# Plonky3/Plonky3-recursion

Measured on AMD Instinct MI355X. Metric: prove_next_layer ms + Poseidon2 perms/s, KoalaBear 2^20-row circuit, 1/8 GPU, lower is better.
Workload: dtype u32 Montgomery (31-bit prime field, degree-4 extension); Poseidon2 hashing as exact integers in f64; 1 GPU; prove_next_layer (verifier-circuit run on the device + prove_all_tables) of the synthetic koala-bear 2^20-row recursion layer: tables const/public/alu/poseidon2/recompose, FRI blowup 4, arity<=4, 54 queries, 15-bit PoW; circuit inputs + NextLayerPrepCache resident in HBM; field=koala-bear, log_height=20, independent_proofs=1, proof_bytes=612900, parallelism=1 independent proofs, one per GPU, no data-path collective

## Files before the change

__graft_entry__.py:

```python
import os
import subprocess
import sys
import time

ROOT = os.path.dirname(os.path.abspath(__file__))
CSRC = os.path.join(ROOT, "plonky3_recursion_amd", "csrc")
LIB = os.path.join(ROOT, "plonky3_recursion_amd", "libp3r_hip.so")
KNOBS_LIB = os.path.join(ROOT, "plonky3_recursion_amd", "knobs", "libp3r_hip.so")
HIP_SOURCES = ["p3r_core.hip", "tu_lde.hip", "tu_open.hip", "tu_fri.hip", "tu_air.hip", "tu_quotient.hip", "tu_logup.hip", "tu_mmcs4.hip", "prep_device.hip"]


def _stale(target, deps):
    if not os.path.exists(target):
        return True
    t = os.path.getmtime(target)
    return any(os.path.getmtime(d) > t for d in deps)


def _deps_of(obj):
    dep = obj + ".d"
    if not os.path.exists(dep):
        return None
    txt = open(dep).read().replace("\\\n", " ")
    return [p for p in txt.split(":", 1)[1].split() if p]


def build():
    hipcc = os.environ.get("HIPCC", "/opt/rocm/bin/hipcc")
    flags = ["-O3", "-std=c++17", "--offload-arch=gfx950", "-fPIC", "-pthread"]
    objdir = os.path.join(CSRC, ".build")
    os.makedirs(objdir, exist_ok=True)
    os.makedirs(os.path.dirname(KNOBS_LIB), exist_ok=True)
    shared = ["prep_device.hip", "tu_open.hip", "tu_fri.hip", "tu_air.hip", "tu_quotient.hip", "tu_logup.hip", "tu_mmcs4.hip"]
    knobbed = ["p3r_core.hip", "tu_lde.hip"]
    units = [(src, src + ".o", []) for src in HIP_SOURCES]
    units += [(src, src.replace(".hip", ".knobs.o"), ["-DP3R_TUNING_KNOBS"]) for src in knobbed]
    test_only = ["tu_prims_test.hip", "tu_p2f_test.hip", "tu_field_test.hip"]
    units += [(src, src.replace(".hip", ".knobs.o"), ["-DP3R_TUNING_KNOBS"]) for src in test_only]
    pending = []
    for src, objname, extra in units:
        obj = os.path.join(objdir, objname)
        deps = _deps_of(obj)
        if deps is None or not all(os.path.exists(d) for d in deps) or _stale(obj, deps):
            pending.append((obj, [hipcc] + flags + extra + ["-MD", "-MF", obj + ".d", "-c", "-o", obj, os.path.join(CSRC, src)]))
    pending.sort(key=lambda job: 0 if "p3r_core" in os.path.basename(job[0]) else 1)
    running, failed = [], None
    max_jobs = max(1, min(len(pending), (os.cpu_count() or 2)))
    while pending or running:
        while pending and len(running) < max_jobs:
            obj, cmd = pending.pop(0)
            running.append((obj, subprocess.Popen(cmd, cwd=CSRC)))
        done = [job for job in running if job[1].poll() is not None]
        if not done:
            time.sleep(0.2)
            continue
        obj, proc = done[0]
        running.remove(done[0])
        if proc.returncode != 0:
            for p in (obj, obj + ".d"):
                if os.path.exists(p):
                    os.remove(p)
            failed = failed or subprocess.CalledProcessError(proc.returncode, proc.args)
    if failed:
        raise failed
    for lib, objs in ((LIB, [s + ".o" for s in HIP_SOURCES]),
                      (KNOBS_LIB, [s.replace(".hip", ".knobs.o") for s in knobbed + test_only] + [s + ".o" for s in shared])):
        paths = [os.path.join(objdir, o) for o in objs]
        if _stale(lib, paths):
            subprocess.run([hipcc] + flags + ["-shared", "-o", lib] + paths, check=True, cwd=CSRC)
    subprocess.run(["make", "-C", os.path.join(ROOT, "oracle")], check=True,
                   stdout=subprocess.DEVNULL)
    subprocess.run(["make", "-C", os.path.join(ROOT, "harness")], check=True,
                   stdout=subprocess.DEVNULL, stderr=subprocess.DEVNULL)
    subprocess.run(["make", "-C", os.path.join(ROOT, "examples")], check=True, stdout=subprocess.DEVNULL)
    chk = os.path.join(ROOT, "tools", "microbench", "zk_fill_check")
    srcs = [chk + ".hip", os.path.join(CSRC, "kernels_zk.hip.h"), os.path.join(CSRC, "zk_rand.h")]
    if not os.path.exists(chk) or any(os.path.getmtime(f) > os.path.getmtime(chk) for f in srcs):
        subprocess.run([hipcc, "--offload-arch=gfx950", "-O3", "-std=c++17", "-w", "-I", CSRC, "-o", chk, chk + ".hip"], check=True)
    if ROOT not in sys.path:
        sys.path.insert(0, ROOT)
    import plonky3_recursion_amd
    from plonky3_recursion_amd import _lib
    _lib.load()


def smoke():
    if ROOT not in sys.path:
        sys.path.insert(0, ROOT)
    sys.path.insert(0, os.path.join(ROOT, "tests"))
    import numpy as np
# ... 66 lines not shown
```

plonky3_recursion_amd/csrc/kernels_fri_reduce.hip.h:

```cpp
#pragma once
#include "kernels_stark.hip.h"

namespace p3r {

template <int DC>
struct FriInvJobT {
  uint32_t* inv;
  uint64_t h;
  int log_h;
  uint32_t w_h;
  uint32_t w_4;
  EW<DC> z;
  uint32_t block0;
};
using FriInvJob = FriInvJobT<4>;
template <class PP, int DC = 4>
__global__ void __launch_bounds__(kBlock)
k_fri_inv_points(const FriInvJobT<DC>* __restrict__ jobs, int n_jobs, uint32_t gen) {
  using F = Fp<PP>;
  using E = typename Chal<PP, DC>::type;
  const int j = find_job(jobs, n_jobs);
  const FriInvJobT<DC>& job = jobs[j];
  const size_t h = job.h, r0 = ((size_t)(blockIdx.x - job.block0) * kBlock + threadIdx.x) * 4;
  if (r0 >= h) return;
  const E z = e4_load<PP, DC>(job.z);
  E x[4], v[4];
  const F x0 = F::raw(gen) * F::raw(job.w_h).pow(bit_reverse((uint32_t)r0, job.log_h));
  const F x2 = x0 * F::raw(job.w_4);
  x[0] = z - E::from_base(x0);
  x[1] = z + E::from_base(x0);
  x[2] = z - E::from_base(x2);
  x[3] = z + E::from_base(x2);
  inv4<PP>(x, v);
  const gptr<uint32_t> inv = as_global(job.inv);
#pragma unroll
  for (int m = 0; m < 4; ++m)
    if (r0 + m < h)
#pragma unroll
      for (int k = 0; k < DC; ++k) inv[(size_t)k * h + r0 + m] = v[m].c[k].v;
}

struct FriVsumJob {
  const uint32_t* vals;
  uint32_t* out;
  int w;
};
template <class PP, int DC = 4>
__global__ void __launch_bounds__(kBlock)
k_fri_vsum(const FriVsumJob* __restrict__ jobs, const uint32_t* __restrict__ apow_tab ) {
  using F = Fp<PP>;
  using E = typename Chal<PP, DC>::type;
  __shared__ uint32_t sh[kBlock / 64][DC];
  const FriVsumJob job = jobs[blockIdx.x];
  const gptr<const uint32_t> vals = as_global(job.vals);
  E acc = E::zero();
  for (int c = threadIdx.x; c < job.w; c += kBlock) {
    E ap, v;
#pragma unroll
    for (int k = 0; k < DC; ++k) {
      ap.c[k] = F::raw(apow_tab[DC * c + k]);
      v.c[k] = F::raw(vals[DC * c + k]);
    }
    acc += ap * v;
  }
  const int lane = threadIdx.x & 63, wave = threadIdx.x >> 6;
#pragma unroll
  for (int k = 0; k < DC; ++k) {
    F x = acc.c[k];
#pragma unroll
    for (int off = 32; off > 0; off >>= 1) x += F::raw(__shfl_down(x.v, off));
    if (lane == 0) sh[wave][k] = x.v;
  }
  __syncthreads();
  if (threadIdx.x < DC) {
    F x = F::zero();
#pragma unroll
    for (int wv = 0; wv < kBlock / 64; ++wv) x += F::raw(sh[wv][threadIdx.x]);
    as_global(job.out)[threadIdx.x] = x.v;
  }
}

template <int DC>
struct FriReduceMatT {
  const uint32_t* mat;
  int w, n_points;
  const uint32_t* inv[2];
  const uint32_t* v[2];
  EW<DC> off[2];
};
using FriReduceMat = FriReduceMatT<4>;
struct FriReduceJob {
  uint32_t* ro;
  uint64_t h;
  uint32_t mat0, n_mats;
  uint32_t block0;
};
template <class PP, int DC = 4>
__global__ void __launch_bounds__(kBlock)
k_fri_reduce_pre(const FriReduceJob* __restrict__ jobs, int n_jobs, const FriReduceMatT<DC>* __restrict__ mats,
                 const uint32_t* __restrict__ apow_tab ) {
  using F = Fp<PP>;
  using E = typename Chal<PP, DC>::type;
  const int j = find_job(jobs, n_jobs);
  const FriReduceJob job = jobs[j];
  const size_t h = job.h, r = (size_t)(blockIdx.x - job.block0) * kBlock + threadIdx.x;
  if (r >= h) return;
  auto apow = [&](int c) {
    E ap;
#pragma unroll
    for (int k = 0; k < DC; ++k) ap.c[k] = F::raw(apow_tab[DC * c + k]);
    return ap;
  };
  E acc = E::zero();
  for (uint32_t m = 0; m < job.n_mats; ++m) {
    const FriReduceMatT<DC>& a = mats[job.mat0 + m];
    const gptr<const uint32_t> mat = as_global(a.mat);
    const int w = a.w;
    E S = E::zero(), S2 = E::zero();
    int c = 0;
    for (; c + 3 < w; c += 4) {
      const F m0 = F::raw(mat[(size_t)c * h + r]), m1 = F::raw(mat[(size_t)(c + 1) * h + r]);
      const F m2 = F::raw(mat[(size_t)(c + 2) * h + r]), m3 = F::raw(mat[(size_t)(c + 3) * h + r]);
      S += E::dot2_base(apow(c), m0, apow(c + 1), m1);
      S2 += E::dot2_base(apow(c + 2), m2, apow(c + 3), m3);
    }
    for (; c + 1 < w; c += 2)
      S += E::dot2_base(apow(c), F::raw(mat[(size_t)c * h + r]), apow(c + 1), F::raw(mat[(size_t)(c + 1) * h + r]));
    if (c < w) S += apow(c) * F::raw(mat[(size_t)c * h + r]);
    S += S2;
    for (int p = 0; p < a.n_points; ++p) {
      E inv;
#pragma unroll
      for (int k = 0; k < DC; ++k) inv.c[k] = F::raw(as_global(a.inv[p])[(size_t)k * h + r]);
      E V;
#pragma unroll
      for (int k = 0; k < DC; ++k) V.c[k] = F::raw(as_global(a.v[p])[k]);
      acc += e4_load<PP, DC>(a.off[p]) * (V - S) * inv;
    }
  }
#pragma unroll
  for (int k = 0; k < DC; ++k) as_global(job.ro)[(size_t)k * h + r] = acc.c[k].v;
}

}
```

plonky3_recursion_amd/csrc/prove_impl.hip.h:

```cpp
#include "host_transcript.h"
#include "kernels_stark.hip.h"
#include "kernels_fri_reduce.hip.h"
#include "kernels_zk.hip.h"
#include "open_impl.hip.h"

struct p3r_prep {
  std::vector<p3r::AirParams> airs;
  std::vector<std::unique_ptr<p3r_dmat>> traces;
  std::vector<std::unique_ptr<p3r_dmat>> evals;
  std::vector<std::unique_ptr<p3r_dmat>> ldes;
  std::vector<size_t> heights;
  int zk_codewords = -1;
  const p3r_dmat* committed(size_t i) const { return evals.empty() ? traces[i].get() : evals[i].get(); }
  std::unique_ptr<p3r_tree> tree;
  std::vector<uint32_t> cap_canonical;
};

namespace {

template <class PP, int DC = 4>
EW<DC> to_e4(const typename Chal<PP, DC>::type& e) { return e4_store<PP, DC>(e); }

template <class PP, int DC = 4>
std::vector<typename Chal<PP, DC>::type> download_ef(p3r_ctx* ctx, const uint32_t* dev, size_t count) {
  std::vector<uint32_t> raw(count * DC);
  P3R_HIP(fetch_small(ctx, dev, raw.size(), raw.data()));
  std::vector<typename Chal<PP, DC>::type> out(count);
  for (size_t i = 0; i < count; ++i)
    for (int k = 0; k < DC; ++k) out[i].c[k] = Fp<PP>::raw(raw[i * DC + k]);
  return out;
}

inline ZkKey zk_key_of(const p3r_ctx* ctx, uint64_t nonce) {
  ZkKey k{};
  for (int i = 0; i < 8; ++i) k.k[i] = ctx->zk_key[i];
  k.nonce_lo = (uint32_t)nonce; k.nonce_hi = (uint32_t)(nonce >> 32);
  return k;
}

template <class PP>
void launch_zk_tiles(p3r_ctx* ctx, std::vector<ZkTileJob>& jobs, const ZkKey& key, const char* family) {
  uint64_t blocks = 0;
  for (auto& j : jobs) {
    if (2 * (uint64_t)(j.w2 | 1u) > kZkTileWords) fail(P3R_EUNSUPPORTED, "ZK fill of a matrix of %u columns", j.w2);
    j.log_tr = zk_tile_log_rows(j.rows, j.w2);
    j.block0 = (uint32_t)blocks;
    blocks += j.rows >> j.log_tr;
  }
  if (blocks >= (uint64_t(1) << 31)) fail(P3R_EUNSUPPORTED, "ZK fill launch of %llu tiles", (unsigned long long)blocks);
  if (!blocks) return;
  DevBuf d_jobs((jobs.size() * sizeof(ZkTileJob) + 3) / 4);
  P3R_HIP(ctx->stage.upload(ctx->stream, d_jobs.p, jobs.data(), jobs.size() * sizeof(ZkTileJob)));
  ProfScope ps(ctx, family);
  hipLaunchKernelGGL(k_zk_fill_tiles<PP>, dim3((unsigned)blocks), dim3(kBlock), 0, ctx->stream, reinterpret_cast<const ZkTileJob*>(d_jobs.p),
                     (int)jobs.size(), key);
// ... 196 lines not shown
  }
  std::vector<uint32_t> cap_mont;
  const ZkKey prep_key = zk_key_of(ctx, 0);
  prep->tree = lde_and_commit<PP>(ctx, items, (int)ctx->cfg.log_blowup, prep->ldes, cap_mont, kSaltRound + ZK_ROUND_PREP, &prep_key);
  prep->cap_canonical.resize(cap_mont.size());
  for (size_t i = 0; i < cap_mont.size(); ++i) prep->cap_canonical[i] = F::raw(cap_mont[i]).to_canonical();
  return prep;
}

template <class PP, int DC>
struct ProofRound {
  using E = typename Chal<PP, DC>::type;
  struct Mat {
    int inst;
    const p3r_dmat *ev, *lde;
    Fp<PP> shift;
    std::vector<E> z;
    size_t job = 0;
    std::vector<std::vector<E>> vals, codewords;
  };
  std::unique_ptr<p3r_tree> own;
  const p3r_tree* tree = nullptr;
  std::vector<uint32_t> cap;
  std::vector<std::unique_ptr<p3r_dmat>> keep, lde;
  std::vector<Mat> mats;
};

template <class PP, int DC>
struct BatchProver {
  using F = Fp<PP>;
  using E = typename Chal<PP, DC>::type;
  using Round = ProofRound<PP, DC>;
  using Mat = typename Round::Mat;
  static constexpr size_t kMaxPhases = 32;

  p3r_ctx* const ctx;
  const p3r_prep* const prep;
  const p3r_dmat* const* const mains;
  const size_t ni;
  const p3r_config& cfg;
  const int log_blowup;
  const int zk, R;
  const ZkKey zk_key;
  std::vector<LookupLayout> layouts;
  std::vector<int> log_n, log_e;
  const F gen = F::generator();
  std::vector<uint32_t> rc_mont;
  HostChallenger<PP, DC> ch;
  ProofWriter<PP, DC> W;
  Round main_round, perm_round, quot_round, rand_round, prep_round;
  LookupChT<DC> lc{};
  std::vector<E> terminals;
  E alpha, zeta;
  DevBuf d_apow, d_fapow;
  Opener<PP, DC> op;
  std::map<std::array<uint64_t, 6>, uint32_t*> inv_cache;
  std::vector<DevBuf> inv_keep;
  std::map<int, std::pair<E, DevBuf>> ros;
  struct Phase { int la; size_t rows; DevBuf folded_in; std::unique_ptr<p3r_tree> tree; std::vector<uint32_t> cap; };
  std::vector<Phase> phases;
  int log_max = 0;
  DevBuf folded, d_tstate, d_phase;
  std::vector<F> commit_pow_witnesses;
  std::vector<E> final_poly;
  F query_pow_witness;
  struct QPath { uint32_t at = 0; const p3r_tree* t = nullptr; };
  struct QRound { std::vector<std::pair<uint32_t, uint32_t>> rows; QPath path; uint32_t tree_shift; };
  struct QPhase { uint32_t sib_at[16]; QPath path; int shift; uint32_t salt_at = 0; };
  std::vector<size_t> indices;
  std::vector<QRound> qrounds;
  std::vector<QPhase> qphases;
  uint32_t words_per_query = 0;
  const uint32_t* gathered = nullptr;

  BatchProver(p3r_ctx* c, const p3r_prep* p, const p3r_dmat* const* m, size_t n, bool canonical_encoding)
      : ctx(c), prep(p), mains(m), ni(n), cfg(c->cfg), log_blowup((int)cfg.log_blowup), zk(cfg.zk ? 1 : 0), R(zk_codewords(cfg)),
        zk_key(zk_key_of(c, (zk || cfg.mmcs_salt_elems) ? c->zk_nonce++ : 0)),
        layouts(n), log_n(n), log_e(n), rc_mont(c->rc_canonical.size()), ch(rc_mont.data()), terminals(n, E::zero()),
        op(c) {
    const int p2w = p2_perm_cols<PP>() + 2;
    for (size_t i = 0; i < ni; ++i) {
      const AirParams& a = prep->airs[i];
      if (mains[i]->h != prep->heights[i])
        fail(P3R_EINVAL, "instance %zu: trace height %zu != preprocessed height %zu", i, mains[i]->h, prep->heights[i]);
      if ((int)mains[i]->w != air_width_of(a, p2w, p2w_perm_cols<PP>() + 4))
        fail(P3R_EINVAL, "instance %zu: trace width %zu, the AIR expects %d", i, mains[i]->w, air_width_of(a, p2w, p2w_perm_cols<PP>() + 4));
      log_n[i] = log2_exact(mains[i]->h, "trace height");
      log_e[i] = log_n[i] + zk;
      layouts[i] = lookup_layout(a, zk);
      if (layouts[i].log_chunks > log_blowup) fail(P3R_EUNSUPPORTED, "quotient domain larger than the LDE (zk %d, log_blowup %d)", zk, log_blowup);
      if ((1 << (layouts[i].log_chunks + zk)) > 8) fail(P3R_EUNSUPPORTED, "more than 8 quotient chunks");
    }
    for (size_t i = 0; i < rc_mont.size(); ++i) rc_mont[i] = F::from_canonical(ctx->rc_canonical[i]).v;
    W.canonical = canonical_encoding;
    prep_round.tree = prep->tree.get();
    for (size_t i = 0; i < ni; ++i) prep_round.mats.push_back({(int)i, prep->committed(i), prep->ldes[i].get(), F::one()});
  }

  std::vector<Round*> rounds() {
    std::vector<Round*> rs;
    for (Round* r : {&rand_round, &main_round, &quot_round, &prep_round, &perm_round})
      if (r->tree) rs.push_back(r);
    return rs;
  }

  const Mat* perm_mat(size_t i) const {
    for (const Mat& m : perm_round.mats)
      if (m.inst == (int)i) return &m;
    return nullptr;
  }

  void commit(Round& r, int zk_round) {
    std::vector<LdeItem> items;
    for (const Mat& m : r.mats) items.push_back({m.ev, (gen * m.shift.inv()).to_canonical()});
    r.own = lde_and_commit<PP>(ctx, items, log_blowup, r.lde, r.cap, kSaltRound + zk_round, &zk_key);
    r.tree = r.own.get();
    for (size_t k = 0; k < r.mats.size(); ++k) r.mats[k].lde = r.lde[k].get();
  }

  void randomise(Round& r, int zk_round) {
    std::vector<const p3r_dmat*> src;
    std::vector<size_t> hs, ws;
    std::vector<uint32_t> keys;
    for (size_t k = 0; k < r.mats.size(); ++k) {
      const p3r_dmat* a = r.mats[k].ev;
      src.push_back(a); hs.push_back(a->h); ws.push_back(a->w); keys.push_back(zk_stream_id(zk_round, k));
    }
    auto rs = zk_randomize<PP>(ctx, src, hs, ws, R, keys, zk_key, false);
    for (size_t k = 0; k < rs.size(); ++k) {
      r.mats[k].ev = rs[k].get();
      r.keep.push_back(std::move(rs[k]));
    }
// ... 197 lines not shown
      P3R_HIP(hipGetLastError());
      k0 += C;
    }
    auto q_odd = coset_lde_batch<PP>(ctx, q_moves, 0), t_odd = coset_lde_batch<PP>(ctx, t_moves, 0);
    std::vector<ZkChunkJob> jobs;
    uint64_t blocks = 0;
    for (size_t k = 0; k < quot_round.mats.size(); ++k) {
      const size_t n = quot_round.mats[k].ev->h;
      auto m = dmat_alloc(2 * n, (size_t)DC + R);
      ZkChunkJob j{};
      j.q = quot_round.mats[k].ev->d; j.q_odd = q_odd[k]->d; j.t_odd = t_odd[k]->d; j.dst = m->d;
      j.n = n; j.log_n = log_n[quot_round.mats[k].inst]; j.DC = DC; j.R = R;
      j.stream = zk_stream_id(ZK_ROUND_QUOTIENT, k);
      j.block0 = (uint32_t)blocks;
      blocks += (uint64_t)(DC + R) * ((2 * n + kBlock - 1) / kBlock);
      jobs.push_back(j);
      quot_round.mats[k].ev = m.get();
      quot_round.keep.push_back(std::move(m));
    }
    if (blocks >= (uint64_t(1) << 31)) fail(P3R_EUNSUPPORTED, "ZK chunk launch of %llu tiles", (unsigned long long)blocks);
    DevBuf d_jobs((jobs.size() * sizeof(ZkChunkJob) + 3) / 4);
    P3R_HIP(ctx->stage.upload(ctx->stream, d_jobs.p, jobs.data(), jobs.size() * sizeof(ZkChunkJob)));
    {
      ProfScope ps(ctx, "zk_chunks");
      hipLaunchKernelGGL(k_zk_chunk<PP>, dim3((unsigned)blocks), dim3(kBlock), 0, ctx->stream,
                         reinterpret_cast<const ZkChunkJob*>(d_jobs.p), (int)jobs.size(), zk_key);
    }
    P3R_HIP(hipGetLastError());
    for (auto& m : q_odd) quot_round.keep.push_back(std::move(m));
    for (auto& m : t_odd) quot_round.keep.push_back(std::move(m));
  }

  void openings() {
    prof_stage(ctx, "openings");
    for (Round* r : rounds())
      for (Mat& m : r->mats) {
        m.z = {zeta};
        if (r == &prep_round || r == &perm_round || (r == &main_round && air_uses_next(prep->airs[m.inst])))
          m.z.push_back(zeta * F::two_adic_generator(log_n[m.inst]));
        m.job = op.open(m.ev->d, m.ev->h, (int)m.ev->w, m.shift, m.z);
      }
    auto all = op.finish();
    launch_inv_points();
    for (Round* r : rounds())
      for (Mat& m : r->mats)
        for (auto& pv : all[m.job]) {
          for (auto& v : pv) ch.observe_ext(v);
          m.vals.emplace_back(pv.begin(), pv.end() - R);
          m.codewords.emplace_back(pv.end() - R, pv.end());
        }
    check_at_zeta();
  }

  static std::array<uint64_t, 6> inv_key(int lh, const E& z) {
    std::array<uint64_t, 6> key{(uint64_t)lh, 0, 0, 0, 0, 0};
    for (int k = 0; k < DC; ++k) key[1 + k] = z.c[k].v;
    return key;
  }

  void launch_inv_points() {
    std::vector<FriInvJobT<DC>> inv_jobs;
    uint32_t inv_blocks = 0;
    for (Round* r : rounds())
      for (const Mat& m : r->mats) {
        const int lh = log_e[m.inst] + log_blowup;
        for (const E& z : m.z) {
          const auto key = inv_key(lh, z);
          if (inv_cache.count(key)) continue;
          inv_keep.emplace_back((size_t)DC << lh);
          FriInvJobT<DC> j{};
          j.inv = inv_keep.back().p;
          j.h = uint64_t(1) << lh;
          j.log_h = lh;
          if (lh < 2) fail(P3R_EINVAL, "FRI: an LDE of fewer than four rows");
          j.w_h = F::two_adic_generator(lh).v;
          j.w_4 = F::two_adic_generator(2).v;
          j.z = to_e4<PP, DC>(z);
          j.block0 = inv_blocks;
          inv_blocks += blocks_for((size_t(1) << lh) / 4);
          inv_jobs.push_back(j);
          inv_cache.emplace(key, j.inv);
        }
      }
    inv_keep.emplace_back((inv_jobs.size() * sizeof(FriInvJobT<DC>) + 3) / 4);
    P3R_HIP(ctx->stage.upload(ctx->stream, inv_keep.back().p, inv_jobs.data(), inv_jobs.size() * sizeof(FriInvJobT<DC>)));
    ProfScope ps(ctx, "fri_inv_points");
    hipLaunchKernelGGL((k_fri_inv_points<PP, DC>), dim3(inv_blocks), dim3(kBlock), 0, ctx->stream,
                       reinterpret_cast<const FriInvJobT<DC>*>(inv_keep.back().p), (int)inv_jobs.size(), gen.v);
    P3R_HIP(hipGetLastError());
  }

  void check_at_zeta() {
    E l_beta_pow[kMaxExtD + 1];
    for (int j = 0; j <= kMaxExtD; ++j) l_beta_pow[j] = e4_load<PP, DC>(lc.beta_pow[j]);
    const E l_prefix = e4_load<PP, DC>(lc.prefix);
    std::vector<std::vector<std::vector<E>>> inst_chunks(ni);
    for (const Mat& m : quot_round.mats) inst_chunks[m.inst].push_back(m.vals[0]);
    static const std::vector<E> empty;
    for (size_t i = 0; i < ni; ++i) {
      const auto& omain = main_round.mats[i].vals;
      const Mat* pm = perm_mat(i);
      ZetaInstance<PP, DC> zi{&omain[0], omain.size() > 1 ? &omain[1] : nullptr, &prep_round.mats[i].vals[0],
                          &prep_round.mats[i].vals[1], pm ? &pm->vals[0] : &empty, pm ? &pm->vals[1] : &empty,
                          &inst_chunks[i], pm ? &terminals[i] : nullptr};
      try {
        check_instance_at_zeta<PP, DC>(prep->airs[i], layouts[i], log_n[i], zi, alpha, zeta, l_prefix, l_beta_pow,
                                   ctx->rc_mont_host.data(), i, zk);
      } catch (const VerifyFailure& e) {
        fail(P3R_EINVAL, "the traces do not satisfy the constraints (%s)", e.what());
      }
    }
    E tsum = E::zero();
    for (const Mat& m : perm_round.mats) tsum += terminals[m.inst];
    if (!tsum.is_zero()) fail(P3R_EINVAL, "the traces do not satisfy the constraints (global lookup sum is not zero)");
  }

  void fri_reduce() {
    prof_stage(ctx, "fri_reduce");
    const E fri_alpha = ch.sample_ext();
    size_t max_w = 1, n_opened = 0;
    for (Round* r : rounds())
      for (const Mat& m : r->mats) { max_w = std::max(max_w, m.lde->w); ++n_opened; }
    std::vector<E> fa_pow(max_w + 1);
    fa_pow[0] = E::one();
    for (size_t c = 1; c <= max_w; ++c) fa_pow[c] = fa_pow[c - 1] * fri_alpha;
    d_fapow.alloc(max_w * DC);
    {
      std::vector<uint32_t> h(max_w * DC);
      for (size_t c = 0; c < max_w; ++c)
        for (int k = 0; k < DC; ++k) h[c * DC + k] = fa_pow[c].c[k].v;
      P3R_HIP(ctx->stage.upload(ctx->stream, d_fapow.p, h.data(), h.size() * 4));
    }
    std::map<int, std::vector<FriReduceMatT<DC>>> by_height;
    std::vector<DevBuf> keep;
    std::vector<FriVsumJob> vsum_jobs;
    DevBuf vsums(2 * DC * n_opened);
    for (Round* r : rounds())
      for (const Mat& m : r->mats) {
        const int lh = log_e[m.inst] + log_blowup;
        auto f = ros.find(lh);
        if (f == ros.end()) f = ros.emplace(lh, std::make_pair(E::one(), DevBuf((size_t)DC << lh))).first;
        FriReduceMatT<DC> a{};
        a.mat = m.lde->d;
        a.w = (int)m.lde->w;
        a.n_points = (int)m.z.size();
        E ap = f->second.first;
        for (size_t p = 0; p < m.z.size(); ++p) {
          a.inv[p] = inv_cache.at(inv_key(lh, m.z[p]));
          a.v[p] = vsums.p + DC * vsum_jobs.size();
          vsum_jobs.push_back({op.values_dev(m.job, (int)p), vsums.p + DC * vsum_jobs.size(), (int)m.ev->w});
          a.off[p] = to_e4<PP, DC>(ap);
          ap *= fa_pow[m.lde->w];
        }
        f->second.first = ap;
        by_height[lh].push_back(a);
      }
    std::vector<FriReduceMatT<DC>> mats;
    std::vector<FriReduceJob> jobs;
    uint32_t blocks = 0;
    for (auto& kv : by_height) {
      FriReduceJob j{};
      j.ro = ros[kv.first].second.p;
      j.h = uint64_t(1) << kv.first;
      j.mat0 = (uint32_t)mats.size();
      j.n_mats = (uint32_t)kv.second.size();
      j.block0 = blocks;
      blocks += blocks_for(size_t(1) << kv.first);
      jobs.push_back(j);
      mats.insert(mats.end(), kv.second.begin(), kv.second.end());
    }
    const size_t b_mats = mats.size() * sizeof(FriReduceMatT<DC>), b_jobs = jobs.size() * sizeof(FriReduceJob),
                 b_vsum = vsum_jobs.size() * sizeof(FriVsumJob);
    const size_t o_jobs = (b_mats + 15) & ~size_t(15), o_vsum = (o_jobs + b_jobs + 15) & ~size_t(15);
    std::vector<unsigned char> blob(o_vsum + b_vsum);
    std::memcpy(blob.data(), mats.data(), b_mats);
    std::memcpy(blob.data() + o_jobs, jobs.data(), b_jobs);
    std::memcpy(blob.data() + o_vsum, vsum_jobs.data(), b_vsum);
    keep.emplace_back((blob.size() + 3) / 4);
    unsigned char* d_blob = reinterpret_cast<unsigned char*>(keep.back().p);
    P3R_HIP(ctx->stage.upload(ctx->stream, d_blob, blob.data(), blob.size()));
    const auto* d_mats = reinterpret_cast<const FriReduceMatT<DC>*>(d_blob);
    const auto* d_jobs = reinterpret_cast<const FriReduceJob*>(d_blob + o_jobs);
    const auto* d_vsum = reinterpret_cast<const FriVsumJob*>(d_blob + o_vsum);
    {
      ProfScope ps(ctx, "fri_reduce");
      hipLaunchKernelGGL((k_fri_vsum<PP, DC>), dim3((unsigned)vsum_jobs.size()), dim3(kBlock), 0, ctx->stream, d_vsum,
                         d_fapow.p);
      hipLaunchKernelGGL((k_fri_reduce_pre<PP, DC>), dim3(blocks), dim3(kBlock), 0, ctx->stream, d_jobs, (int)jobs.size(),
                         d_mats, d_fapow.p);
    }
    P3R_HIP(hipGetLastError());
  }

  void fri_commit_phase() {
    prof_stage(ctx, "fri_commit_phase");
    std::vector<int> heights;
    for (auto& kv : ros) heights.push_back(kv.first);
    std::sort(heights.rbegin(), heights.rend());
    log_max = heights[0];
    const int log_final = (int)cfg.log_final_poly_len + log_blowup;
    folded = std::move(ros[log_max].second);
    size_t next_h = 1;
    int log_cur = log_max;
    const bool device_transcript = cfg.cap_height == 0 && cfg.commit_pow_bits == 0 && ch.in_buf.empty();
    d_tstate.alloc(P2_WIDTH);
    d_phase.alloc((DC + P2_DIGEST) * kMaxPhases);
    uint32_t* const d_betas = d_phase.p;
    uint32_t* const d_caps = d_phase.p + DC * kMaxPhases;
    if (device_transcript) {
      uint32_t st[P2_WIDTH];
      for (int k = 0; k < P2_WIDTH; ++k) st[k] = ch.state[k].v;
      P3R_HIP(ctx->stage.upload(ctx->stream, d_tstate.p, st, sizeof st));
    }
    while (log_cur > log_final) {
      int log_next = next_h < heights.size() ? heights[next_h] : -1;
      int la = fri_log_arity(ctx->fri_log_arities, phases.size(), (int)cfg.max_log_arity, log_cur, log_final, log_next);
      if (la < 0) fail(P3R_EINVAL, "fri_log_arities does not fit the proof: phase %zu at height 2^%d", phases.size(), log_cur);
      if (la > 4) fail(P3R_EUNSUPPORTED, "max_log_arity > 4 is not supported");
      const size_t arity = size_t(1) << la, rows = (size_t(1) << log_cur) >> la;
      Phase ph{la, rows};
      commit_phase_leaves(ph, log_cur);
      const size_t pi = phases.size();
      if (pi >= kMaxPhases) fail(P3R_EUNSUPPORTED, "more than %zu FRI commit phases", kMaxPhases);
      TranscriptStep step{d_tstate.p, d_betas + DC * pi, d_caps + P2_DIGEST * pi};
      step.dc = DC;
      mmcs_build_levels<PP>(ctx, ph.tree.get(), nullptr, device_transcript ? &step : nullptr);
      if (device_transcript) {
        if (!step.done)
          hipLaunchKernelGGL(k_fri_transcript_step<PP>, dim3(1), dim3(64), 0, ctx->stream, ph.tree->layers.back().p,
                             step.state, step.beta, step.cap, ctx->rc.p, ctx->p2_diag.p, DC);
      } else {
        ph.cap = mmcs_cap_mont(ctx, ph.tree.get());
        for (uint32_t v : ph.cap) ch.observe(F::raw(v));
        commit_pow_witnesses.push_back(grind_witness<PP>(ctx, ch, (int)cfg.commit_pow_bits));
        const E beta = ch.sample_ext();
        uint32_t bw[DC];
        for (int k = 0; k < DC; ++k) bw[k] = beta.c[k].v;
        P3R_HIP(ctx->stage.upload(ctx->stream, d_betas + DC * pi, bw, sizeof bw));
      }
      DevBuf out(DC * rows);
      FriFoldArgs fa{};
      fa.in = folded.p; fa.out = out.p; fa.rows = rows; fa.log_rows = log_cur - la;
      fa.beta = d_betas + DC * pi;
      const bool roll = next_h < heights.size() && heights[next_h] == log_cur - la;
      fa.roll = roll ? ros[heights[next_h]].second.p : nullptr;
      fa.w_inv = F::two_adic_generator(log_cur).inv().v;
      const F omega = F::two_adic_generator(la);
      for (int s = 0; s < la; ++s) {
        F om_s = omega.pow(uint64_t(1) << s);
        for (int j = 0; j < (int)(arity >> (s + 1)); ++j)
          fa.tw_inv[s][j] = om_s.pow(bit_reverse(2 * j, la - s)).inv().v;
      }
      fa.neg_half = (-(F::from_canonical(2).inv())).v;
      {
        ProfScope ps(ctx, "fri_fold");
        static constexpr void (*kFold[4])(FriFoldArgs) = {k_fri_fold<PP, DC, 1>, k_fri_fold<PP, DC, 2>, k_fri_fold<PP, DC, 3>,
                                                          k_fri_fold<PP, DC, 4>};
        hipLaunchKernelGGL(kFold[la - 1], dim3(blocks_for(rows)), dim3(kBlock), 0, ctx->stream, fa);
      }
      P3R_HIP(hipGetLastError());
      if (roll) ++next_h;
      ph.folded_in = std::move(folded);
      folded = std::move(out);
      log_cur -= la;
      phases.push_back(std::move(ph));
    }
    if (next_h != heights.size()) fail(P3R_EINVAL, "FRI: an input height was never rolled in");
    final_polynomial(log_cur, device_transcript);
    for (auto& c : final_poly) ch.observe_ext(c);
    for (auto& ph : phases) ch.observe(F::from_canonical((uint32_t)ph.la));
    query_pow_witness = grind_witness<PP>(ctx, ch, (int)cfg.query_pow_bits);
  }

  void commit_phase_leaves(Phase& ph, int log_cur) {
    const size_t arity = size_t(1) << ph.la, rows = ph.rows, n_in = size_t(1) << log_cur;
    if ((int)cfg.cap_height > log_cur - ph.la)
      fail(P3R_EINVAL, "cap_height %d exceeds the height of FRI commit phase %zu (2^%d rows)", (int)cfg.cap_height,
           phases.size(), log_cur - ph.la);
    ph.tree = std::make_unique<p3r_tree>();
    mmcs_begin(ctx, ph.tree.get(), {rows});
    std::vector<const uint32_t*> cols;
    for (size_t j = 0; j < arity; ++j)
      for (int k = 0; k < DC; ++k) cols.push_back(folded.p + (size_t)k * n_in + j);
    if (cfg.mmcs_salt_elems) {
      const uint32_t S = cfg.mmcs_salt_elems;
      p3r_tree& T = *ph.tree;
      T.salt_elems = (int)S; T.phase_salt_stride = arity; T.phase_rows = rows;
      T.phase_salts.alloc((size_t)S * n_in);
      std::vector<ZkTileJob> tj(1);
      tj[0].dst = T.phase_salts.p; tj[0].rows = rows; tj[0].w2 = S; tj[0].mode = 1; tj[0].stride = (uint32_t)arity;
      tj[0].stream = zk_stream_id(kSaltRoundFri, phases.size());
      launch_zk_tiles<PP>(ctx, tj, zk_key, "mmcs_salts");
      for (uint32_t c = 0; c < S; ++c) cols.push_back(T.phase_salts.p + (size_t)c * n_in);
    }
    mmcs_hash_rows_strided<PP>(ctx, ph.tree.get(), cols, rows, arity);
  }

  void final_polynomial(int log_cur, bool device_transcript) {
// ... 253 lines not shown
```

Before: 27.42 ms.

## Compute FRI reduced openings on the trace domain and extend by LDE

For large non-zk matrices with unit shift, the FRI quotient sum is evaluated on the trace domain in natural order instead of on the blowup-sized LDE. The result, a few extension columns, is then extended with a coset LDE. Any remaining LDE-domain matrices are accumulated on top through a new init pointer. This cuts the reads of wide LDE matrices by the blowup factor, at the cost of an extra small LDE, a second reduce launch and separate inverse-point tables.

```diff
diff --git a/__graft_entry__.py b/__graft_entry__.py
--- a/__graft_entry__.py
+++ b/__graft_entry__.py
@@ -35,7 +35,7 @@
     knobbed = ["p3r_core.hip", "tu_lde.hip"]
     units = [(src, src + ".o", []) for src in HIP_SOURCES]
     units += [(src, src.replace(".hip", ".knobs.o"), ["-DP3R_TUNING_KNOBS"]) for src in knobbed]
-    test_only = ["tu_prims_test.hip", "tu_p2f_test.hip", "tu_field_test.hip"]
+    test_only = ["tu_prims_test.hip", "tu_p2f_test.hip", "tu_field_test.hip", "tu_fri_trace_test.hip"]
     units += [(src, src.replace(".hip", ".knobs.o"), ["-DP3R_TUNING_KNOBS"]) for src in test_only]
     pending = []
     for src, objname, extra in units:
diff --git a/plonky3_recursion_amd/csrc/fri_reduce_impl.hip.h b/plonky3_recursion_amd/csrc/fri_reduce_impl.hip.h
--- /dev/null
+++ b/plonky3_recursion_amd/csrc/fri_reduce_impl.hip.h
@@ -0,0 +1,207 @@
+#pragma once
+#include <array>
+#include <cstring>
+#include <map>
+
+#include "kernels_fri_reduce.hip.h"
+#include "profile.h"
+#include "tu_api.h"
+
+namespace p3r {
+
+constexpr size_t kFriTraceMinRows = size_t(1) << 17;
+
+template <class PP, int DC>
+struct FriReducer {
+  using F = Fp<PP>;
+  using E = typename Chal<PP, DC>::type;
+  struct Item {
+    const p3r_dmat *ev, *lde;
+    F shift;
+    int lh;
+    std::vector<E> z;
+    const uint32_t* vals[2];
+  };
+  enum Domain : uint64_t { LDE = 0, TRACE = 1 };
+
+  p3r_ctx* const ctx;
+  const int log_blowup;
+  const bool zk;
+  const size_t min_trace_rows;
+  bool use_trace = false;
+  std::map<std::array<uint64_t, 7>, const uint32_t*> inv_cache;
+  std::vector<DevBuf> keep;
+  std::vector<std::unique_ptr<p3r_dmat>> keep_mats;
+
+  FriReducer(p3r_ctx* c, int lb, bool z, size_t min_rows) : ctx(c), log_blowup(lb), zk(z), min_trace_rows(min_rows) {}
+
+  static unsigned blocks_of(size_t n) { return (unsigned)((n + kBlock - 1) / kBlock); }
+
+  bool eligible(const Item& m) const {
+    return !zk && m.shift == F::one() && m.ev->h >= 4 && (m.ev->h << log_blowup) == m.lde->h && m.ev->w == m.lde->w &&
+           m.lde->h == (size_t(1) << m.lh);
+  }
+  bool on_trace(const Item& m) const { return use_trace && eligible(m); }
+  static std::array<uint64_t, 7> inv_key(Domain d, int log_h, const E& z) {
+    std::array<uint64_t, 7> key{(uint64_t)d, (uint64_t)log_h, 0, 0, 0, 0, 0};
+    for (int k = 0; k < DC; ++k) key[2 + k] = z.c[k].v;
+    return key;
+  }
+
+  void launch_inv_points(const std::vector<Item>& items) {
+    std::vector<FriInvJobT<DC>> jobs[2];
+    uint32_t blocks[2] = {0, 0};
+    use_trace = false;
+    for (const Item& m : items) use_trace = use_trace || (eligible(m) && m.ev->h >= min_trace_rows);
+    for (const Item& m : items) {
+      if (m.lh < 2) fail(P3R_EINVAL, "FRI: an LDE of fewer than four rows");
+      const Domain d = on_trace(m) ? TRACE : LDE;
+      const int log_h = d == TRACE ? m.lh - log_blowup : m.lh;
+      for (const E& z : m.z) {
+        const auto key = inv_key(d, log_h, z);
+        if (inv_cache.count(key)) continue;
+        keep.emplace_back((size_t)DC << log_h);
+        FriInvJobT<DC> j{};
+        j.inv = keep.back().p;
+        j.h = uint64_t(1) << log_h;
+        j.log_h = log_h;
+        j.w_h = F::two_adic_generator(log_h).v;
+        j.w_4 = F::two_adic_generator(2).v;
+        j.z = e4_store<PP, DC>(z);
+        j.block0 = blocks[d];
+        blocks[d] += blocks_of((size_t(1) << log_h) / 4);
+        jobs[d].push_back(j);
+        inv_cache.emplace(key, j.inv);
+      }
+    }
+    const size_t b0 = jobs[0].size() * sizeof(FriInvJobT<DC>), b1 = jobs[1].size() * sizeof(FriInvJobT<DC>);
+    if (b0 + b1 == 0) return;
+    std::vector<unsigned char> blob(b0 + b1);
+    if (b0) std::memcpy(blob.data(), jobs[0].data(), b0);
+    if (b1) std::memcpy(blob.data() + b0, jobs[1].data(), b1);
+    keep.emplace_back((blob.size() + 3) / 4);
+    unsigned char* d_blob = reinterpret_cast<unsigned char*>(keep.back().p);
+    P3R_HIP(ctx->stage.upload(ctx->stream, d_blob, blob.data(), blob.size()));
+    ProfScope ps(ctx, "fri_inv_points");
+    if (b0)
+      hipLaunchKernelGGL((k_fri_inv_points<PP, DC, false>), dim3(blocks[0]), dim3(kBlock), 0, ctx->stream,
+                         reinterpret_cast<const FriInvJobT<DC>*>(d_blob), (int)jobs[0].size(), F::generator().v);
+    if (b1)
+      hipLaunchKernelGGL((k_fri_inv_points<PP, DC, true>), dim3(blocks[1]), dim3(kBlock), 0, ctx->stream,
+                         reinterpret_cast<const FriInvJobT<DC>*>(d_blob + b0), (int)jobs[1].size(), F::one().v);
+    P3R_HIP(hipGetLastError());
+  }
+
+  std::map<int, DevBuf> reduce(const std::vector<Item>& items, const E& alpha) {
+    size_t max_w = 1;
+    for (const Item& m : items) max_w = std::max(max_w, m.lde->w);
+    std::vector<E> apow(max_w + 1);
+    apow[0] = E::one();
+    for (size_t c = 1; c <= max_w; ++c) apow[c] = apow[c - 1] * alpha;
+    keep.emplace_back(max_w * DC);
+    uint32_t* const d_apow = keep.back().p;
+    {
+      std::vector<uint32_t> h(max_w * DC);
+      for (size_t c = 0; c < max_w; ++c)
+        for (int k = 0; k < DC; ++k) h[c * DC + k] = apow[c].c[k].v;
+      P3R_HIP(ctx->stage.upload(ctx->stream, d_apow, h.data(), h.size() * 4));
+    }
+    struct Height { E a = E::one(); std::vector<FriReduceMatT<DC>> set[2]; };
+    std::map<int, Height> heights;
+    std::vector<FriVsumJob> vsum_jobs;
+    keep.emplace_back(2 * DC * items.size());
+    uint32_t* const vsums = keep.back().p;
+    for (const Item& m : items) {
+      Height& H = heights[m.lh];
+      const Domain d = on_trace(m) ? TRACE : LDE;
+      FriReduceMatT<DC> a{};
+      a.mat = d == TRACE ? m.ev->d : m.lde->d;
+      a.w = (int)m.lde->w;
+      a.n_points = (int)m.z.size();
+      for (size_t p = 0; p < m.z.size(); ++p) {
+        a.inv[p] = inv_cache.at(inv_key(d, d == TRACE ? m.lh - log_blowup : m.lh, m.z[p]));
+        a.v[p] = vsums + DC * vsum_jobs.size();
+        vsum_jobs.push_back({m.vals[p], vsums + DC * vsum_jobs.size(), (int)m.ev->w});
+        a.off[p] = e4_store<PP, DC>(H.a);
+        H.a *= apow[m.lde->w];
+      }
+      H.set[d].push_back(a);
+    }
+    std::map<int, DevBuf> ros;
+    std::vector<FriReduceMatT<DC>> mats;
+    std::vector<FriReduceJob> jobs[2];
+    uint32_t blocks[2] = {0, 0};
+    std::vector<LdeItem> lde_items;
+    std::vector<int> lde_heights;
+    auto add_job = [&](Domain d, int log_h, uint32_t* ro, const std::vector<FriReduceMatT<DC>>& set) {
+      FriReduceJob j{};
+      j.ro = ro;
+      j.h = uint64_t(1) << log_h;
+      j.mat0 = (uint32_t)mats.size();
+      j.n_mats = (uint32_t)set.size();
+      j.block0 = blocks[d];
+      blocks[d] += blocks_of(size_t(1) << log_h);
+      jobs[d].push_back(j);
+      mats.insert(mats.end(), set.begin(), set.end());
+    };
+    for (auto& kv : heights) {
+      if (kv.second.set[TRACE].empty()) continue;
+      keep_mats.push_back(dmat_alloc(size_t(1) << (kv.first - log_blowup), DC));
+      add_job(TRACE, kv.first - log_blowup, keep_mats.back()->d, kv.second.set[TRACE]);
+      lde_items.push_back({keep_mats.back().get(), F::generator().to_canonical()});
+      lde_heights.push_back(kv.first);
+    }
+    for (auto& kv : heights) {
+      if (kv.second.set[LDE].empty()) continue;
+      add_job(LDE, kv.first, nullptr, kv.second.set[LDE]);
+    }
+    auto bind_residual = [&] {
+      for (FriReduceJob& j : jobs[LDE]) {
+        const int lh = log2_exact(j.h, "LDE height");
+        auto f = ros.find(lh);
+        if (f == ros.end()) f = ros.emplace(lh, DevBuf((size_t)DC << lh)).first;
+        else j.init = f->second.p;
+        j.ro = f->second.p;
+      }
+    };
+    const bool split = !lde_items.empty();
+    if (!split) bind_residual();
+    const Domain first = split ? TRACE : LDE;
+    const size_t b_mats = mats.size() * sizeof(FriReduceMatT<DC>), b_jobs = jobs[first].size() * sizeof(FriReduceJob),
+                 b_vsum = vsum_jobs.size() * sizeof(FriVsumJob);
+    const size_t o_jobs = (b_mats + 15) & ~size_t(15), o_vsum = (o_jobs + b_jobs + 15) & ~size_t(15);
+    std::vector<unsigned char> blob(o_vsum + b_vsum);
+    std::memcpy(blob.data(), mats.data(), b_mats);
+    if (b_jobs) std::memcpy(blob.data() + o_jobs, jobs[first].data(), b_jobs);
+    std::memcpy(blob.data() + o_vsum, vsum_jobs.data(), b_vsum);
+    keep.emplace_back((blob.size() + 3) / 4);
+    unsigned char* d_blob = reinterpret_cast<unsigned char*>(keep.back().p);
+    P3R_HIP(ctx->stage.upload(ctx->stream, d_blob, blob.data(), blob.size()));
+    const auto* d_mats = reinterpret_cast<const FriReduceMatT<DC>*>(d_blob);
+    {
+      ProfScope ps(ctx, "fri_reduce");
+      if (!vsum_jobs.empty())
+        hipLaunchKernelGGL((k_fri_vsum<PP, DC>), dim3((unsigned)vsum_jobs.size()), dim3(kBlock), 0, ctx->stream,
+                           reinterpret_cast<const FriVsumJob*>(d_blob + o_vsum), d_apow);
+      if (!jobs[first].empty())
+        hipLaunchKernelGGL((k_fri_reduce_pre<PP, DC>), dim3(blocks[first]), dim3(kBlock), 0, ctx->stream,
+                           reinterpret_cast<const FriReduceJob*>(d_blob + o_jobs), (int)jobs[first].size(), d_mats, d_apow);
+    }
+    P3R_HIP(hipGetLastError());
+    if (!split) return ros;
+    auto ext = coset_lde_batch<PP>(ctx, lde_items, log_blowup);
+    for (size_t i = 0; i < ext.size(); ++i) ros[lde_heights[i]] = std::move(ext[i]->buf);
+    if (!jobs[LDE].empty()) {
+      bind_residual();
+      keep.emplace_back((jobs[LDE].size() * sizeof(FriReduceJob) + 3) / 4);
+      P3R_HIP(ctx->stage.upload(ctx->stream, keep.back().p, jobs[LDE].data(), jobs[LDE].size() * sizeof(FriReduceJob)));
+      ProfScope ps(ctx, "fri_reduce");
+      hipLaunchKernelGGL((k_fri_reduce_pre<PP, DC>), dim3(blocks[LDE]), dim3(kBlock), 0, ctx->stream,
+                         reinterpret_cast<const FriReduceJob*>(keep.back().p), (int)jobs[LDE].size(), d_mats, d_apow);
+      P3R_HIP(hipGetLastError());
+    }
+    return ros;
+  }
+};
+
+}
diff --git a/plonky3_recursion_amd/csrc/kernels_fri_reduce.hip.h b/plonky3_recursion_amd/csrc/kernels_fri_reduce.hip.h
--- a/plonky3_recursion_amd/csrc/kernels_fri_reduce.hip.h
+++ b/plonky3_recursion_amd/csrc/kernels_fri_reduce.hip.h
@@ -14,7 +14,7 @@
   uint32_t block0;
 };
 using FriInvJob = FriInvJobT<4>;
-template <class PP, int DC = 4>
+template <class PP, int DC = 4, bool NATURAL = false>
 __global__ void __launch_bounds__(kBlock)
 k_fri_inv_points(const FriInvJobT<DC>* __restrict__ jobs, int n_jobs, uint32_t gen) {
   using F = Fp<PP>;
@@ -25,12 +25,22 @@
   if (r0 >= h) return;
   const E z = e4_load<PP, DC>(job.z);
   E x[4], v[4];
-  const F x0 = F::raw(gen) * F::raw(job.w_h).pow(bit_reverse((uint32_t)r0, job.log_h));
-  const F x2 = x0 * F::raw(job.w_4);
-  x[0] = z - E::from_base(x0);
-  x[1] = z + E::from_base(x0);
-  x[2] = z - E::from_base(x2);
-  x[3] = z + E::from_base(x2);
+  if constexpr (NATURAL) {
+    const F w = F::raw(job.w_h);
+    F xm = F::raw(gen) * w.pow(r0);
+#pragma unroll
+    for (int m = 0; m < 4; ++m) {
+      x[m] = z - E::from_base(xm);
+      xm *= w;
+    }
+  } else {
+    const F x0 = F::raw(gen) * F::raw(job.w_h).pow(bit_reverse((uint32_t)r0, job.log_h));
+    const F x2 = x0 * F::raw(job.w_4);
+    x[0] = z - E::from_base(x0);
+    x[1] = z + E::from_base(x0);
+    x[2] = z - E::from_base(x2);
+    x[3] = z + E::from_base(x2);
+  }
   inv4<PP>(x, v);
   const gptr<uint32_t> inv = as_global(job.inv);
 #pragma unroll
@@ -91,6 +101,7 @@
 using FriReduceMat = FriReduceMatT<4>;
 struct FriReduceJob {
   uint32_t* ro;
+  const uint32_t* init;
   uint64_t h;
   uint32_t mat0, n_mats;
   uint32_t block0;
@@ -112,6 +123,9 @@
     return ap;
   };
   E acc = E::zero();
+  if (job.init)
+#pragma unroll
+    for (int k = 0; k < DC; ++k) acc.c[k] = F::raw(as_global(job.init)[(size_t)k * h + r]);
   for (uint32_t m = 0; m < job.n_mats; ++m) {
     const FriReduceMatT<DC>& a = mats[job.mat0 + m];
     const gptr<const uint32_t> mat = as_global(a.mat);
diff --git a/plonky3_recursion_amd/csrc/prove_impl.hip.h b/plonky3_recursion_amd/csrc/prove_impl.hip.h
--- a/plonky3_recursion_amd/csrc/prove_impl.hip.h
+++ b/plonky3_recursion_amd/csrc/prove_impl.hip.h
@@ -1,6 +1,6 @@
 #include "host_transcript.h"
 #include "kernels_stark.hip.h"
-#include "kernels_fri_reduce.hip.h"
+#include "fri_reduce_impl.hip.h"
 #include "kernels_zk.hip.h"
 #include "open_impl.hip.h"
 
@@ -303,11 +303,10 @@
   LookupChT<DC> lc{};
   std::vector<E> terminals;
   E alpha, zeta;
-  DevBuf d_apow, d_fapow;
+  DevBuf d_apow;
   Opener<PP, DC> op;
-  std::map<std::array<uint64_t, 6>, uint32_t*> inv_cache;
-  std::vector<DevBuf> inv_keep;
-  std::map<int, std::pair<E, DevBuf>> ros;
+  FriReducer<PP, DC> fri;
+  std::map<int, DevBuf> ros;
   struct Phase { int la; size_t rows; DevBuf folded_in; std::unique_ptr<p3r_tree> tree; std::vector<uint32_t> cap; };
   std::vector<Phase> phases;
   int log_max = 0;
@@ -328,7 +327,7 @@
       : ctx(c), prep(p), mains(m), ni(n), cfg(c->cfg), log_blowup((int)cfg.log_blowup), zk(cfg.zk ? 1 : 0), R(zk_codewords(cfg)),
         zk_key(zk_key_of(c, (zk || cfg.mmcs_salt_elems) ? c->zk_nonce++ : 0)),
         layouts(n), log_n(n), log_e(n), rc_mont(c->rc_canonical.size()), ch(rc_mont.data()), terminals(n, E::zero()),
-        op(c) {
+        op(c), fri(c, log_blowup, zk != 0, kFriTraceMinRows) {
     const int p2w = p2_perm_cols<PP>() + 2;
     for (size_t i = 0; i < ni; ++i) {
       const AirParams& a = prep->airs[i];
@@ -632,43 +631,19 @@
     check_at_zeta();
   }
 
-  static std::array<uint64_t, 6> inv_key(int lh, const E& z) {
-    std::array<uint64_t, 6> key{(uint64_t)lh, 0, 0, 0, 0, 0};
-    for (int k = 0; k < DC; ++k) key[1 + k] = z.c[k].v;
-    return key;
-  }
-
-  void launch_inv_points() {
-    std::vector<FriInvJobT<DC>> inv_jobs;
-    uint32_t inv_blocks = 0;
+  std::vector<typename FriReducer<PP, DC>::Item> fri_items(bool with_values) {
+    std::vector<typename FriReducer<PP, DC>::Item> items;
     for (Round* r : rounds())
       for (const Mat& m : r->mats) {
-        const int lh = log_e[m.inst] + log_blowup;
-        for (const E& z : m.z) {
-          const auto key = inv_key(lh, z);
-          if (inv_cache.count(key)) continue;
-          inv_keep.emplace_back((size_t)DC << lh);
-          FriInvJobT<DC> j{};
-          j.inv = inv_keep.back().p;
-          j.h = uint64_t(1) << lh;
-          j.log_h = lh;
-          if (lh < 2) fail(P3R_EINVAL, "FRI: an LDE of fewer than four rows");
-          j.w_h = F::two_adic_generator(lh).v;
-          j.w_4 = F::two_adic_generator(2).v;
-          j.z = to_e4<PP, DC>(z);
-          j.block0 = inv_blocks;
-          inv_blocks += blocks_for((size_t(1) << lh) / 4);
-          inv_jobs.push_back(j);
-          inv_cache.emplace(key, j.inv);
-        }
-      }
-    inv_keep.emplace_back((inv_jobs.size() * sizeof(FriInvJobT<DC>) + 3) / 4);
-    P3R_HIP(ctx->stage.upload(ctx->stream, inv_keep.back().p, inv_jobs.data(), inv_jobs.size() * sizeof(FriInvJobT<DC>)));
-    ProfScope ps(ctx, "fri_inv_points");
-    hipLaunchKernelGGL((k_fri_inv_points<PP, DC>), dim3(inv_blocks), dim3(kBlock), 0, ctx->stream,
-                       reinterpret_cast<const FriInvJobT<DC>*>(inv_keep.back().p), (int)inv_jobs.size(), gen.v);
-    P3R_HIP(hipGetLastError());
-  }
+        typename FriReducer<PP, DC>::Item it{m.ev, m.lde, m.shift, log_e[m.inst] + log_blowup, m.z, {nullptr, nullptr}};
+        if (with_values)
+          for (size_t p = 0; p < m.z.size(); ++p) it.vals[p] = op.values_dev(m.job, (int)p);
+        items.push_back(std::move(it));
+      }
+    return items;
+  }
+
+  void launch_inv_points() { fri.launch_inv_points(fri_items(false)); }
 
   void check_at_zeta() {
     E l_beta_pow[kMaxExtD + 1];
@@ -698,78 +673,7 @@
   void fri_reduce() {
     prof_stage(ctx, "fri_reduce");
     const E fri_alpha = ch.sample_ext();
-    size_t max_w = 1, n_opened = 0;
-    for (Round* r : rounds())
-      for (const Mat& m : r->mats) { max_w = std::max(max_w, m.lde->w); ++n_opened; }
-    std::vector<E> fa_pow(max_w + 1);
-    fa_pow[0] = E::one();
-    for (size_t c = 1; c <= max_w; ++c) fa_pow[c] = fa_pow[c - 1] * fri_alpha;
-    d_fapow.alloc(max_w * DC);
-    {
-      std::vector<uint32_t> h(max_w * DC);
-      for (size_t c = 0; c < max_w; ++c)
-        for (int k = 0; k < DC; ++k) h[c * DC + k] = fa_pow[c].c[k].v;
-      P3R_HIP(ctx->stage.upload(ctx->stream, d_fapow.p, h.data(), h.size() * 4));
-    }
-    std::map<int, std::vector<FriReduceMatT<DC>>> by_height;
-    std::vector<DevBuf> keep;
-    std::vector<FriVsumJob> vsum_jobs;
-    DevBuf vsums(2 * DC * n_opened);
-    for (Round* r : rounds())
-      for (const Mat& m : r->mats) {
-        const int lh = log_e[m.inst] + log_blowup;
-        auto f = ros.find(lh);
-        if (f == ros.end()) f = ros.emplace(lh, std::make_pair(E::one(), DevBuf((size_t)DC << lh))).first;
-        FriReduceMatT<DC> a{};
-        a.mat = m.lde->d;
-        a.w = (int)m.lde->w;
-        a.n_points = (int)m.z.size();
-        E ap = f->second.first;
-        for (size_t p = 0; p < m.z.size(); ++p) {
-          a.inv[p] = inv_cache.at(inv_key(lh, m.z[p]));
-          a.v[p] = vsums.p + DC * vsum_jobs.size();
-          vsum_jobs.push_back({op.values_dev(m.job, (int)p), vsums.p + DC * vsum_jobs.size(), (int)m.ev->w});
-          a.off[p] = to_e4<PP, DC>(ap);
-          ap *= fa_pow[m.lde->w];
-        }
-        f->second.first = ap;
-        by_height[lh].push_back(a);
-      }
-    std::vector<FriReduceMatT<DC>> mats;
-    std::vector<FriReduceJob> jobs;
-    uint32_t blocks = 0;
-    for (auto& kv : by_height) {
-      FriReduceJob j{};
-      j.ro = ros[kv.first].second.p;
-      j.h = uint64_t(1) << kv.first;
-      j.mat0 = (uint32_t)mats.size();
-      j.n_mats = (uint32_t)kv.second.size();
-      j.block0 = blocks;
-      blocks += blocks_for(size_t(1) << kv.first);
-      jobs.push_back(j);
-      mats.insert(mats.end(), kv.second.begin(), kv.second.end());
-    }
-    const size_t b_mats = mats.size() * sizeof(FriReduceMatT<DC>), b_jobs = jobs.size() * sizeof(FriReduceJob),
-                 b_vsum = vsum_jobs.size() * sizeof(FriVsumJob);
-    const size_t o_jobs = (b_mats + 15) & ~size_t(15), o_vsum = (o_jobs + b_jobs + 15) & ~size_t(15);
-    std::vector<unsigned char> blob(o_vsum + b_vsum);
-    std::memcpy(blob.data(), mats.data(), b_mats);
-    std::memcpy(blob.data() + o_jobs, jobs.data(), b_jobs);
-    std::memcpy(blob.data() + o_vsum, vsum_jobs.data(), b_vsum);
-    keep.emplace_back((blob.size() + 3) / 4);
-    unsigned char* d_blob = reinterpret_cast<unsigned char*>(keep.back().p);
-    P3R_HIP(ctx->stage.upload(ctx->stream, d_blob, blob.data(), blob.size()));
-    const auto* d_mats = reinterpret_cast<const FriReduceMatT<DC>*>(d_blob);
-    const auto* d_jobs = reinterpret_cast<const FriReduceJob*>(d_blob + o_jobs);
-    const auto* d_vsum = reinterpret_cast<const FriVsumJob*>(d_blob + o_vsum);
-    {
-      ProfScope ps(ctx, "fri_reduce");
-      hipLaunchKernelGGL((k_fri_vsum<PP, DC>), dim3((unsigned)vsum_jobs.size()), dim3(kBlock), 0, ctx->stream, d_vsum,
-                         d_fapow.p);
-      hipLaunchKernelGGL((k_fri_reduce_pre<PP, DC>), dim3(blocks), dim3(kBlock), 0, ctx->stream, d_jobs, (int)jobs.size(),
-                         d_mats, d_fapow.p);
-    }
-    P3R_HIP(hipGetLastError());
+    ros = fri.reduce(fri_items(true), fri_alpha);
   }
 
   void fri_commit_phase() {
@@ -779,7 +683,7 @@
     std::sort(heights.rbegin(), heights.rend());
     log_max = heights[0];
     const int log_final = (int)cfg.log_final_poly_len + log_blowup;
-    folded = std::move(ros[log_max].second);
+    folded = std::move(ros[log_max]);
     size_t next_h = 1;
     int log_cur = log_max;
     const bool device_transcript = cfg.cap_height == 0 && cfg.commit_pow_bits == 0 && ch.in_buf.empty();
@@ -823,7 +727,7 @@
       fa.in = folded.p; fa.out = out.p; fa.rows = rows; fa.log_rows = log_cur - la;
       fa.beta = d_betas + DC * pi;
       const bool roll = next_h < heights.size() && heights[next_h] == log_cur - la;
-      fa.roll = roll ? ros[heights[next_h]].second.p : nullptr;
+      fa.roll = roll ? ros[heights[next_h]].p : nullptr;
       fa.w_inv = F::two_adic_generator(log_cur).inv().v;
       const F omega = F::two_adic_generator(la);
       for (int s = 0; s < la; ++s) {
```

Result: faster. 26.96 ms (median of 6 runs) (-1.7%).
